# hpc4cmb/flacarray

Hardware: AMD Instinct MI355X
Metric: Msamples/s encode+decode, 4096ch x 1Msamp int32 (higher is better)
Workload: dtype int32

## Files before the change

flacarray_amd/csrc/encode_fused.hpp:

```cpp
#pragma once
#include "encode_kernels.hpp"
#include "quantize_kernels.hpp"

namespace fa {

constexpr int kFSmpWords = 65 * 32;
#ifndef FA_F_SCANW
#define FA_F_SCANW 4
#endif
#ifndef FA_F_RING
#define FA_F_RING 1024
#endif
constexpr int kFRingWords = FA_F_RING;
constexpr int kFRingMask = kFRingWords - 1;
constexpr int kFRingBlocks = kFRingWords / 64;
constexpr int kFRowBlocks = 12;
static_assert(kFRingBlocks - kFRowBlocks - 1 >= 1, "the ring must hold the longest row and a partial block beside what waits to be flushed");
constexpr int kFWaveWords = kFSmpWords + kFRingWords + 4 + 16;
constexpr int kFWaves = 4;
constexpr int kFCrcSlice = 1024;
constexpr int kFCrcXpow = 520;
#ifndef FA_F_SLEEP
#define FA_F_SLEEP 8
#endif
#ifndef FA_F_WBATCH
#define FA_F_WBATCH 4
#endif
#ifndef FA_F_CEIL
#define FA_F_CEIL 1
#endif
#ifndef FA_F_BFLY_N
#define FA_F_BFLY_N 1
#endif
#ifndef FA_F_PARKN
#define FA_F_PARKN 32
#endif
#ifndef FA_F_PARKBLK
#define FA_F_PARKBLK 1
#endif
#ifndef FA_F_PARK
#define FA_F_PARK 1
#endif
#ifndef FA_F_WAVES
#define FA_F_WAVES 3
#endif
constexpr uint32_t kLbSpinLimit = 1u << 22;

struct FusedArgs {
    const int32_t* data;
    const float* f_offsets;
    const float* f_gains;
    int64_t n_stream, stream_size, nframes, total_frames;
    int32_t max_lpc_order, max_porder, precision, pmax_full;
    int32_t tail_bs;
    double escale_full;
    const float* win;
    const uint4* hdr;
    uint8_t* blob;
    int64_t capacity;
    int64_t hb;
    uint32_t* frame_bytes;
    int64_t* frame_abs;
    FrameInfo* info;
    uint32_t* ticket;
    uint32_t* size_pub;
// ... 165 lines not shown
                if ((uint32_t)lane < cnt) {
                    const uint64_t off = prefix + (incl - mine) + (uint64_t)(i / nf + 1u) * (uint64_t)a.hb;
                    __hip_atomic_store(a.off_pub + i, (unsigned long long)off, __ATOMIC_RELAXED, __HIP_MEMORY_SCOPE_AGENT);
#ifdef FA_TIMELINE
                    if (a.info) a.info[i].porder = (int32_t)(uint32_t)__builtin_amdgcn_s_memrealtime();
#endif
                }
                prefix += (uint32_t)__builtin_amdgcn_readlane((int)incl, 63);
                adv += cnt;
            }
            open = open && (cnt == 64u);
        }
        pos += adv;
        if (adv == 0) {
            __builtin_amdgcn_s_sleep(4);
            if (++idle > kLbSpinLimit) {
                if (lane == 0) atomicOr(a.err, 4);
                return;
            }
        } else {
            idle = 0;
        }
    }
    if (lane == 0) *a.total = (int64_t)(prefix + (uint64_t)a.n_stream * (uint64_t)a.hb);
}

#if defined(FA_UNIT_FUSED) || !defined(FA_SPLIT_UNITS)
template <int MLO, bool F32IN = false>
__global__ __launch_bounds__(256) __attribute__((amdgpu_waves_per_eu(MLO > 8 ? 2 : FA_F_WAVES, MLO > 8 ? 2 : FA_F_WAVES))) void encode_fused_kernel(FusedArgs a) {
    static_assert(MLO > 0, "levels 0-2 (fixed predictors, 1152-sample blocks) use the slot path");
    __shared__ __attribute__((aligned(16))) int32_t lds_all[kFWaves * kFWaveWords];
    __shared__ __attribute__((aligned(16))) uint16_t crc_s[kFCrcSlice];
    __shared__ uint32_t ticket_s;

    const int tid = threadIdx.x;
    const int lane = tid & 63;
    const int wave = __builtin_amdgcn_readfirstlane(tid >> 6);
    for (int i = tid; i < kFCrcSlice / 2; i += 256) reinterpret_cast<uint32_t*>(crc_s)[i] = reinterpret_cast<const uint32_t*>(a.crc_tab)[i];
    if (tid == 0) ticket_s = __hip_atomic_fetch_add(a.ticket, 1u, __ATOMIC_RELAXED, __HIP_MEMORY_SCOPE_AGENT);
    __syncthreads();
    const uint32_t ticket = (uint32_t)__builtin_amdgcn_readfirstlane((int)ticket_s);
    if (ticket == 0) {
        if (wave == 0) fused_scanner(a, lane);
        return;
    }
    const int64_t g = (int64_t)(ticket - 1) * kFWaves + wave;
    if (g >= a.total_frames) return;

    int32_t* smp = lds_all + wave * kFWaveWords;
    uint32_t* ring = reinterpret_cast<uint32_t*>(smp + kFSmpWords);
    uint8_t* kpar = reinterpret_cast<uint8_t*>(smp + kFSmpWords + kFRingWords + 4);
    uint32_t* scr = ring;

    const int64_t s = (int64_t)((uint32_t)g / (uint32_t)a.nframes);
    const int64_t f = g - s * a.nframes;
    if (f == a.nframes - 1 && a.tail_bs != kMaxBlock) return;
    constexpr int bs = kMaxBlock;
    const int32_t* src = a.data + (s * a.stream_size + f * (int64_t)bs);
    float q_off = 0.0f, q_gain = 0.0f;
    if constexpr (F32IN) { q_off = a.f_offsets[s]; q_gain = a.f_gains[s]; }
    auto load_row = [&](int j) __attribute__((always_inline)) {
        const int4 v = reinterpret_cast<const int4*>(src)[64 * j + lane];
        if constexpr (F32IN)
            return make_int4(quantise_f32(__int_as_float(v.x), q_off, q_gain), quantise_f32(__int_as_float(v.y), q_off, q_gain),
                             quantise_f32(__int_as_float(v.z), q_off, q_gain), quantise_f32(__int_as_float(v.w), q_off, q_gain));
        else
            return v;
    };
    const float* win = a.win;
    const uint4 fhe = a.hdr[f];
    const uint32_t fh_bits = 32u + ((fhe.w >> 8) & 0xFFu) + ((fhe.w >> 16) & 0xFFu) + (fhe.w >> 24) + 8u;

#define FA_IMAGE_ADDRS                                                                  \
    const int ln_ = lane_id_opaque();                                                   \
    const int K = fsmp_unit(ln_ + 1, 0);                                                \
    const int rowbase = fsmp_unit((ln_ >> 3) + 1, ln_ & 7);                             \
    const int hist7 = fsmp_unit(ln_, 7), hist6 = fsmp_unit(ln_, 6), hist5 = fsmp_unit(ln_, 5); \
    (void)K; (void)rowbase; (void)hist7; (void)hist6; (void)hist5
    constexpr int tailA7 = 32 * 64 + 4 * (7 ^ (64 & 7)), tailA6 = 32 * 64 + 4 * (6 ^ (64 & 7)), tailA5 = 32 * 64 + 4 * (5 ^ (64 & 7));

    FA_STAMP_INIT;
#ifdef FA_TIMELINE
    const uint32_t tl_start_ = (uint32_t)__builtin_amdgcn_s_memrealtime();
#endif
    int4 Bv[8];
    uint32_t orv = 0;
    int mn, mx;
    {
        FA_IMAGE_ADDRS;
        int4 hi[8], lo[8];
// ... 44 lines not shown
        mn >>= wasted;
        mx >>= wasted;
    }
    const bool narrow = (mn >= -(1 << 24)) && (mx < (1 << 24));
    lds_fence();

    FA_STAMP(0);
    const uint64_t verbatim_bits = 8 + (uint64_t)wasted + (uint64_t)bs * (uint64_t)bps;
    int type = 1;
    int order = 0, porder = 0, shift = 0, precision = 0;
    int kbest = 0;
    bool img_is_residual = false;
    bool win_small_l = false, win_small_f = false;
    int fo = -1;
    int32_t qkeep[MLO];
#pragma unroll
    for (int j = 0; j < MLO; ++j) qkeep[j] = 0;
    const int pmax_geo = a.pmax_full;
    auto pmax_for = [&](int pred_order) __attribute__((always_inline)) {
        int pm = pmax_geo;
        while (pm > 0 && (bs >> pm) <= pred_order) pm--;
        return pm;
    };

    auto hist_b = [&](const int4& own, const int4& tail) __attribute__((always_inline)) {
        int4 h;
        h.x = dpp_wave_shr1(tail.x, own.x);
        h.y = dpp_wave_shr1(tail.y, own.y);
        h.z = dpp_wave_shr1(tail.z, own.z);
        h.w = dpp_wave_shr1(tail.w, own.w);
        return h;
    };

    if (__builtin_expect(is_const, 0)) {
        type = 0;
    } else {
        uint64_t best_bits = verbatim_bits;
        double tot0 = 0.0, tot1 = 0.0, tot2 = 0.0, tot3 = 0.0, tot4 = 0.0;
        double mx0 = 0.0, mx1 = 0.0, mx2 = 0.0, mx3 = 0.0, mx4 = 0.0;
        uint64_t hA0 = 0, hA1 = 0, hA2 = 0, hA3 = 0, hA4 = 0;
        double dA0 = 0.0, dA1 = 0.0, dA2 = 0.0, dA3 = 0.0, dA4 = 0.0;
        if (__builtin_expect(narrow, 1)) {
            FA_IMAGE_ADDRS;
            const uint32_t BIAS = 0x80000000u;
            uint32_t s0 = 0, s1 = 0, s2 = 0, s3 = 0, s4 = 0;
            int p1, pe1, pe2, pe3;
            auto seed = [&](const int4& hh) __attribute__((always_inline)) {
                p1 = hh.w;
                pe1 = hh.w - hh.z;
                pe2 = pe1 - (hh.z - hh.y);
                pe3 = pe2 - ((hh.z - hh.y) - (hh.y - hh.x));
            };
            auto group = [&](auto mask_tag, const int4& xv, int gi0) __attribute__((always_inline)) {
                constexpr bool MASK = decltype(mask_tag)::value;
                const int xs[4] = {xv.x, xv.y, xv.z, xv.w};
#pragma unroll
                for (int e = 0; e < 4; ++e) {
                    const int x = xs[e];
                    const int e1 = x - p1, e2 = e1 - pe1, e3 = e2 - pe2;
                    const uint32_t xb = (uint32_t)x ^ BIAS;
                    const uint32_t n0 = sad_u32(xb, BIAS, s0);
                    const uint32_t n1 = sad_u32(xb, (uint32_t)p1 ^ BIAS, s1);
                    const uint32_t n2 = sad_u32((uint32_t)e1 ^ BIAS, (uint32_t)pe1 ^ BIAS, s2);
                    const uint32_t n3 = sad_u32((uint32_t)e2 ^ BIAS, (uint32_t)pe2 ^ BIAS, s3);
                    const uint32_t n4 = sad_u32((uint32_t)e3 ^ BIAS, (uint32_t)pe3 ^ BIAS, s4);
                    if constexpr (MASK) {
                        const int gi = gi0 + e;
                        s0 = n0;
                        s1 = (gi >= 1) ? n1 : s1;
                        s2 = (gi >= 2) ? n2 : s2;
// ... 58 lines not shown
                    mx1 = __builtin_fmax(mx1, a1);
                    mx2 = __builtin_fmax(mx2, a2);
                    mx3 = __builtin_fmax(mx3, a3);
                    mx4 = __builtin_fmax(mx4, a4);
                    p1 = xd; pe1 = e1; pe2 = e2; pe3 = e3;
                }
            };
            seed(*reinterpret_cast<const int4*>(&smp[hist7]));
#pragma unroll 1
            for (int t = 0; t < 8; ++t) group(*reinterpret_cast<const int4*>(&smp[K ^ (4 * t)]), 32 * lane + 4 * t);
            dA0 = tot0; dA1 = tot1; dA2 = tot2; dA3 = tot3; dA4 = tot4;
            seed(hist_b(Bv[7], *reinterpret_cast<const int4*>(&smp[tailA7])));
#pragma unroll
            for (int t = 0; t < 8; ++t) group(Bv[t], 4096);
        }
        FA_STAMP(1);
        {
            double tsum[5] = {tot0, tot1, tot2, tot3, tot4};
            wave_sum_butterfly_n<5>(tsum);
            const double T0 = tsum[0], T1 = tsum[1], T2 = tsum[2], T3 = tsum[3], T4 = tsum[4];
            double M0 = 0.0, M1 = 0.0, M2 = 0.0, M3 = 0.0, M4 = 0.0;
            if (!narrow) {
                M0 = wave_max_f64(mx0); M1 = wave_max_f64(mx1); M2 = wave_max_f64(mx2); M3 = wave_max_f64(mx3);
                M4 = wave_max_f64(mx4);
            }
            const double lim = 2147483647.0;
            double smallest = 1.8446744073709552e19;
            if (M0 <= lim && T0 < smallest) { fo = 0; smallest = T0; }
            if (M1 <= lim && T1 < smallest) { fo = 1; smallest = T1; }
            if (M2 <= lim && T2 < smallest) { fo = 2; smallest = T2; }
            if (M3 <= lim && T3 < smallest) { fo = 3; smallest = T3; }
            if (M4 <= lim && T4 < smallest) { fo = 4; smallest = T4; }
        }
        uint64_t fixA, fixB;
        if (narrow) {
            const uint64_t tA = (fo == 0) ? hA0 : (fo == 1) ? hA1 : (fo == 2) ? hA2 : (fo == 3) ? hA3 : hA4;
            const double tt = (fo == 0) ? tot0 : (fo == 1) ? tot1 : (fo == 2) ? tot2 : (fo == 3) ? tot3 : tot4;
            fixA = tA;
            fixB = (uint64_t)tt - tA;
        } else {
            const double tA = (fo == 0) ? dA0 : (fo == 1) ? dA1 : (fo == 2) ? dA2 : (fo == 3) ? dA3 : dA4;
            const double tt = (fo == 0) ? tot0 : (fo == 1) ? tot1 : (fo == 2) ? tot2 : (fo == 3) ? tot3 : tot4;
            fixA = (uint64_t)tA;
            fixB = (uint64_t)(tt - tA);
        }
        int po_fix = 0, k_fix = 0;
        const int pmax_fix = pmax_for(fo < 0 ? 0 : fo);
        const bool small_fix = __all((fixA < (1u << 24)) && (fixB < (1u << 24)));
        win_small_f = small_fix;
        const bool fuse_search = fo >= 0 && pmax_fix <= 5 && a.max_lpc_order > 0 && small_fix;
        uint64_t est_fix = 0;
        auto apply_fixed = [&]() __attribute__((always_inline)) {
            if (est_fix < best_bits) {
                best_bits = est_fix;
                type = 2;
                order = fo;
                porder = po_fix;
                kbest = k_fix;
            }
        };
        if (__builtin_expect(fo >= 0 && !fuse_search, 0)) {
            uint64_t rb;
            if (pmax_fix <= 5 && small_fix) {
                SplitRiceSearch fs;
                fs.start((uint32_t)fixA, (uint32_t)fixB, fo, pmax_fix, lane);
                fs.gather(); fs.params(); fs.totals();
#pragma unroll
                for (int o = 5; o >= 0; --o) fs.order(o);
                po_fix = fs.bpo; k_fix = fs.kb; rb = fs.best;
            } else {
                rb = split_rice_search_slow(fixA, fixB, fo, pmax_fix, lane, &po_fix, &k_fix);
            }
            est_fix = 8 + (uint64_t)wasted + (uint64_t)fo * (uint64_t)bps + rb;
            apply_fixed();
        }

        FA_STAMP(2);
        int mlo = a.max_lpc_order;
        if (__builtin_expect(mlo > 0, 1)) {
            FA_IMAGE_ADDRS;
            double acc[MLO + 1];
#pragma unroll
            for (int j = 0; j <= MLO; ++j) acc[j] = 0.0;
            SplitRiceSearch fs;
            if (fuse_search) fs.start((uint32_t)fixA, (uint32_t)fixB, fo, pmax_fix, lane);
            double hist[MLO];
            struct WinV { double w[4]; };
            auto load_win = [&](int i0) __attribute__((always_inline)) {
                const float4 f = *reinterpret_cast<const float4*>(win + i0);
                WinV v;
                v.w[0] = (double)f.x; v.w[1] = (double)f.y; v.w[2] = (double)f.z; v.w[3] = (double)f.w;
                return v;
            };
            auto lag_group = [&](const int4& xv, const WinV& wv) __attribute__((always_inline)) {
                const int xs[4] = {xv.x, xv.y, xv.z, xv.w};
#pragma unroll
                for (int e = 0; e < 4; ++e) {
                    const double d = (double)xs[e] * wv.w[e];
                    acc[0] = __builtin_fma(d, d, acc[0]);
#pragma unroll
                    for (int j = 0; j < MLO; ++j) acc[j + 1] = __builtin_fma(d, hist[j], acc[j + 1]);
#pragma unroll
                    for (int j = MLO - 1; j > 0; --j) hist[j] = hist[j - 1];
                    hist[0] = d;
                }
            };
            auto search_stage = [&](int tt) __attribute__((always_inline)) {
                if (!fuse_search) return;
                if (tt == 1) fs.gather();
                if (tt == 3) fs.params();
                if (tt == 5) fs.totals();
                if (tt >= 7 && tt <= 12) fs.order(12 - tt);
// ... 36 lines not shown
#pragma unroll
                for (int t = 0; t < 4; ++t) Bv[4 + t] = pk[64 * t];
            }
#endif
            {
                const int g0 = 2048 + 32 * lane;
                const int4 h7 = hist_b(Bv[7], *reinterpret_cast<const int4*>(&smp[tailA7]));
                const int4 h6 = hist_b(Bv[6], *reinterpret_cast<const int4*>(&smp[tailA6]));
                int4 h5 = make_int4(0, 0, 0, 0);
                if constexpr (MLO > 8) h5 = hist_b(Bv[5], *reinterpret_cast<const int4*>(&smp[tailA5]));
                const int hs[12] = {h7.w, h7.z, h7.y, h7.x, h6.w, h6.z, h6.y, h6.x, h5.w, h5.z, h5.y, h5.x};
#pragma unroll
                for (int j = 0; j < MLO; ++j) hist[j] = (double)hs[j] * (double)win[g0 - 1 - j];
#pragma unroll
                for (int tb = 0; tb < 8; tb += FA_F_WBATCH) {
                    WinV wv[FA_F_WBATCH];
#pragma unroll
                    for (int t = 0; t < FA_F_WBATCH; ++t) wv[t] = load_win(g0 + 4 * (tb + t));
#pragma unroll
                    for (int t = 0; t < FA_F_WBATCH; ++t) {
                        lag_group(Bv[tb + t], wv[t]);
                        search_stage(8 + tb + t);
                    }
                    __builtin_amdgcn_sched_barrier(0);
                }
            }
            FA_STAMP(4);
            if (fuse_search) {
                po_fix = fs.bpo;
                k_fix = fs.kb;
                est_fix = 8 + (uint64_t)wasted + (uint64_t)fo * (uint64_t)bps + (uint64_t)fs.best;
                apply_fixed();
            }
            double autoc[MLO + 1];
#if FA_F_BFLY_N
#pragma unroll
            for (int j = 0; j <= MLO; ++j) autoc[j] = acc[j];
            wave_sum_butterfly_n<MLO + 1>(autoc);
#else
#pragma unroll
            for (int j = 0; j <= MLO; ++j) autoc[j] = wave_sum_butterfly(acc[j]);
#endif

            FA_STAMP(5);
            if (__builtin_expect(autoc[0] != 0.0, 1)) {
                float* coef = reinterpret_cast<float*>(scr);
                double* err = reinterpret_cast<double*>(scr + 160);
                int* meta = reinterpret_cast<int*>(scr + 220);
                if (lane == 0) meta[0] = levinson<MLO>(autoc, mlo, coef, err);
                lds_fence();
                const int usable = meta[0];
                int prec = a.precision;
                int lo;
                {
                    double mybits = 1e300;
                    if (lane < usable) {
                        const double e = err[lane];
                        const double error_scale = a.escale_full;
                        double bpsv;
                        if (e > 0.0) {
                            bpsv = 0.5 * det_log2(error_scale * e);
                            if (!(bpsv >= 0.0)) bpsv = 0.0;
                        } else if (e < 0.0) {
                            bpsv = 1e32;
                        } else {
                            bpsv = 0.0;
                        }
                        mybits = bpsv * (double)(bs - (lane + 1)) + (double)((lane + 1) * (bps + prec));
                    }
                    double bestb = 4294967295.0;
                    int bi = 0;
#pragma unroll
                    for (int o = 0; o < MLO; ++o) {
                        const double b = readlane_f64(mybits, o);
                        if (o < usable && b < bestb) { bestb = b; bi = o; }
                    }
                    lo = bi + 1;
                }
                if (bps <= 17) {
                    const int limp = 32 - bps - ilog2_u64((uint64_t)lo);
                    if (prec > limp) prec = limp;
                }
                int sh = 0;
                int32_t qreg[MLO];
#pragma unroll
                for (int j = 0; j < MLO; ++j) qreg[j] = 0;
                int ok = 0;
                if (prec >= 2) ok = (quantize_coefs_t<MLO>(coef + (lo - 1) * MLO, lo, prec, qreg, &sh) == 0) ? 1 : 0;
                ok = __builtin_amdgcn_readfirstlane(ok);
                sh = __builtin_amdgcn_readfirstlane(sh);
#pragma unroll
                for (int j = 0; j < MLO; ++j) qreg[j] = __builtin_amdgcn_readfirstlane(qreg[j]);
                FA_STAMP(6);
                if (__builtin_expect(ok != 0, 1)) {
                    FA_IMAGE_ADDRS;
                    const double scale = bitsd((uint64_t)(1023 - sh) << 52);
                    double qd[MLO];
#pragma unroll
                    for (int j = 0; j < MLO; ++j) qd[j] = (double)qreg[j] * scale;
                    double tlA = 0.0, tlB = 0.0;
                    double hx[MLO];
                    const int4 a7 = *reinterpret_cast<const int4*>(&smp[hist7]), a6 = *reinterpret_cast<const int4*>(&smp[hist6]);
                    const int4 a5 = *reinterpret_cast<const int4*>(&smp[hist5]);
                    const int4 b7 = hist_b(Bv[7], *reinterpret_cast<const int4*>(&smp[tailA7]));
                    const int4 b6 = hist_b(Bv[6], *reinterpret_cast<const int4*>(&smp[tailA6]));
                    int4 b5 = make_int4(0, 0, 0, 0);
                    if constexpr (MLO > 8) b5 = hist_b(Bv[5], *reinterpret_cast<const int4*>(&smp[tailA5]));
                    lds_fence();
                    auto fold_f64 = [&](double r) __attribute__((always_inline)) {
                        return (int)(uint32_t)__builtin_fabs(__builtin_fma(r, 2.0, 0.5));
                    };
                    auto res_group = [&](auto mask_tag, const int4& xv, int gi0, double& tl) __attribute__((always_inline)) {
                        constexpr bool MASK = decltype(mask_tag)::value;
                        const int xs[4] = {xv.x, xv.y, xv.z, xv.w};
                        int rs[4];
#pragma unroll
                        for (int e = 0; e < 4; ++e) {
                            const double xd = (double)xs[e];
#if FA_F_CEIL
                            double t = xd;
#pragma unroll
                            for (int j = 0; j < MLO; ++j) t = __builtin_fma(-qd[j], hx[j], t);
                            const double r = fa_ceil(t);
#else
                            double sum = 0.0;
#pragma unroll
                            for (int j = 0; j < MLO; ++j) sum = __builtin_fma(qd[j], hx[j], sum);
                            const double pred = fa_floor(sum);
                            const double r = xd - pred;
#endif
                            if constexpr (MASK) {
                                const bool v = (gi0 + e >= lo);
                                tl += v ? fa_fabs(r) : 0.0;
                                rs[e] = v ? fold_f64(r) : xs[e];
                            } else {
                                tl += fa_fabs(r);
                                rs[e] = fold_f64(r);
                            }
#pragma unroll
                            for (int j = MLO - 1; j > 0; --j) hx[j] = hx[j - 1];
                            hx[0] = xd;
                        }
                        return make_int4(rs[0], rs[1], rs[2], rs[3]);
                    };
                    constexpr int kWarmGroups = (MLO + 3) / 4;
                    {
                        const int hs[12] = {a7.w, a7.z, a7.y, a7.x, a6.w, a6.z, a6.y, a6.x, a5.w, a5.z, a5.y, a5.x};
#pragma unroll
                        for (int j = 0; j < MLO; ++j) hx[j] = (double)hs[j];
#pragma unroll
                        for (int t = 0; t < 8; ++t) {
                            int4* px = reinterpret_cast<int4*>(&smp[K ^ (4 * t)]);
                            if (t < kWarmGroups) *px = res_group(std::true_type{}, *px, 32 * lane + 4 * t, tlA);
                            else *px = res_group(std::false_type{}, *px, 0, tlA);
                        }
                    }
                    {
                        const int hs[12] = {b7.w, b7.z, b7.y, b7.x, b6.w, b6.z, b6.y, b6.x, b5.w, b5.z, b5.y, b5.x};
#pragma unroll
                        for (int j = 0; j < MLO; ++j) hx[j] = (double)hs[j];
#pragma unroll
                        for (int t = 0; t < 8; ++t) Bv[t] = res_group(std::false_type{}, Bv[t], 0, tlB);
                    }
                    FA_STAMP(7);
                    img_is_residual = true;
                    const int pmax = pmax_for(lo);
                    int po_l = 0, k_l = 0;
                    uint64_t rbits;
                    const bool small_l = __all((tlA < 16777216.0) && (tlB < 16777216.0));
                    bool lpc_in_range = true;
                    if (__builtin_expect(!small_l, 0)) {
                        bool hit = false;
#pragma unroll 1
                        for (int t = 0; t < 8; ++t) {
                            const int4 ra = *reinterpret_cast<const int4*>(&smp[K ^ (4 * t)]);
                            const int ras[4] = {ra.x, ra.y, ra.z, ra.w};
#pragma unroll
                            for (int e = 0; e < 4; ++e) hit = hit || ((32 * lane + 4 * t + e >= lo) && (uint32_t)ras[e] == 0xffffffffu);
                        }
#pragma unroll
                        for (int t = 0; t < 8; ++t)
                            hit = hit || (uint32_t)Bv[t].x == 0xffffffffu || (uint32_t)Bv[t].y == 0xffffffffu || (uint32_t)Bv[t].z == 0xffffffffu ||
                                  (uint32_t)Bv[t].w == 0xffffffffu;
                        lpc_in_range = !__any(hit);
                    }
                    win_small_l = small_l;
                    if (pmax <= 5 && small_l) {
                        SplitRiceSearch ls;
                        ls.start((uint32_t)tlA, (uint32_t)tlB, lo, pmax, lane);
                        ls.gather(); ls.params(); ls.totals();
#pragma unroll
                        for (int o = 5; o >= 0; --o) ls.order(o);
                        po_l = ls.bpo; k_l = ls.kb; rbits = ls.best;
                    } else {
                        rbits = split_rice_search_slow((uint64_t)tlA, (uint64_t)tlB, lo, pmax, lane, &po_l, &k_l);
                    }
                    if (lpc_in_range) {
                        const uint64_t est = 8 + (uint64_t)wasted + 4 + 5 + (uint64_t)lo * (uint64_t)(prec + bps) + rbits;
                        if (est < best_bits) {
                            best_bits = est;
                            type = 3;
                            order = lo;
                            porder = po_l;
                            kbest = k_l;
                            shift = sh;
                            precision = prec;
#pragma unroll
                            for (int j = 0; j < MLO; ++j) qkeep[j] = qreg[j];
                        }
                    }
                }
                lds_fence();
            }
        }
    }

    FA_STAMP(8);
    const int lane_w = lane_id_opaque();
    auto reload_image = [&]() __attribute__((always_inline)) {
        FA_IMAGE_ADDRS;
#pragma unroll 1
        for (int half = 1; half >= 0; --half) {
#pragma unroll
            for (int j = 0; j < 8; ++j) {
                int4 v = load_row(8 * half + j);
                v.x >>= wasted; v.y >>= wasted; v.z >>= wasted; v.w >>= wasted;
                *reinterpret_cast<int4*>(&smp[rowbase + 256 * j]) = v;
            }
            if (half == 1) {
#pragma unroll
                for (int t = 0; t < 8; ++t) Bv[t] = *reinterpret_cast<const int4*>(&smp[K ^ (4 * t)]);
            }
        }
        lds_fence();
    };
    if (__builtin_expect(type == 2, 0)) {
        if (img_is_residual) {
            reload_image();
            img_is_residual = false;
        }
        {
            FA_IMAGE_ADDRS;
            const int4 ha = *reinterpret_cast<const int4*>(&smp[hist7]);
            const int4 hb2 = hist_b(Bv[7], *reinterpret_cast<const int4*>(&smp[tailA7]));
            lds_fence();
            int64_t x1, x2, x3, x4;
            auto fgroup = [&](const int4& xv, int gi0) __attribute__((always_inline)) {
                const int xs[4] = {xv.x, xv.y, xv.z, xv.w};
                int rs[4];
#pragma unroll
                for (int e = 0; e < 4; ++e) {
                    const int64_t x0 = xs[e];
                    int64_t r;
                    if (order == 0) r = x0;
                    else if (order == 1) r = x0 - x1;
                    else if (order == 2) r = x0 - 2 * x1 + x2;
                    else if (order == 3) r = x0 - 3 * x1 + 3 * x2 - x3;
                    else r = x0 - 4 * x1 + 6 * x2 - 4 * x3 + x4;
                    rs[e] = (gi0 + e >= order) ? rice_fold((int)r) : xs[e];
                    x4 = x3; x3 = x2; x2 = x1; x1 = x0;
                }
                return make_int4(rs[0], rs[1], rs[2], rs[3]);
            };
            x1 = ha.w; x2 = ha.z; x3 = ha.y; x4 = ha.x;
#pragma unroll 1
            for (int t = 0; t < 8; ++t) {
                int4* px = reinterpret_cast<int4*>(&smp[K ^ (4 * t)]);
                *px = fgroup(*px, 32 * lane_w + 4 * t);
            }
            x1 = hb2.w; x2 = hb2.z; x3 = hb2.y; x4 = hb2.x;
#pragma unroll
// ... 40 lines not shown
        };
        if (__builtin_expect((type == 3) ? win_small_l : win_small_f, 1)) size_lane(std::false_type{});
        else size_lane(std::true_type{});
        bitsA += (8 - kWarmGroupsS) * 4 * (kA + 1u);
        bitsB += 32u * (kB + 1u);
        if (((uint32_t)lane_w & (cpp - 1u)) == 0u || cpp > 64u) {
            if (cpp <= 64u) { bitsA += (uint32_t)plen; bitsB += (uint32_t)plen; }
            else if (lane_w == 0) bitsA += (uint32_t)plen;
        }
        uint32_t rA = bitsA, rB = bitsB;
        rA += (uint32_t)xchg_i32<0>((int)rA); rB += (uint32_t)xchg_i32<0>((int)rB);
        rA += (uint32_t)xchg_i32<1>((int)rA); rB += (uint32_t)xchg_i32<1>((int)rB);
        rA += (uint32_t)xchg_i32<2>((int)rA); rB += (uint32_t)xchg_i32<2>((int)rB);
        const bool row_over = __any((rA > (uint32_t)kRowCapBits) || (rB > (uint32_t)kRowCapBits));
        const uint64_t exact = 6 + wave_sum_u64((uint64_t)bitsA + bitsB) + 8 + (uint64_t)wasted + (uint64_t)order * (uint64_t)bps +
                               ((type == 3) ? (4 + 5 + (uint64_t)order * (uint64_t)precision) : 0);
        if (row_over || exact > verbatim_bits) {
            type = 1;
            order = 0;
            porder = 0;
        }
        sub_bits = (uint32_t)exact;
    }
    if (type == 0) sub_bits = 8u + (uint32_t)wasted + (uint32_t)bps;
    if (type == 1) sub_bits = (uint32_t)verbatim_bits;
    const uint32_t total_bytes = ((fh_bits + sub_bits + 7u) >> 3) + 2u;
    const uint32_t L = total_bytes - 2u;

    FA_STAMP(9);
    const uint32_t F = (uint32_t)a.total_frames;
    const uint32_t gu = (uint32_t)g;
#ifdef FA_TIMELINE
    if (lane_w == 0 && a.info) {
        a.info[g].wasted = (int32_t)tl_start_;
        a.info[g].shift = (int32_t)(uint32_t)__builtin_amdgcn_s_memrealtime();
        __builtin_amdgcn_s_waitcnt(0);
    }
#endif
    if (lane_w == 0) {
        __hip_atomic_store(a.size_pub + gu, 0x80000000u | total_bytes, __ATOMIC_RELAXED, __HIP_MEMORY_SCOPE_AGENT);
        a.frame_bytes[g] = total_bytes;
    }
    (void)F;
#ifndef FA_TIMELINE
    if (lane_w == 0 && a.info) {
        FrameInfo fi;
        fi.type = type;
        fi.order = (type >= 2) ? order : 0;
        fi.porder = (type >= 2) ? porder : 0;
        fi.wasted = wasted;
        fi.shift = (type == 3) ? shift : 0;
        fi.precision = (type == 3) ? precision : 0;
        fi.nbytes = (int32_t)total_bytes;
        fi.blocksize = bs;
        a.info[g] = fi;
    }
#endif

#ifdef FA_F_ANALYSIS_ONLY
    if (lane_w == 0) a.frame_abs[g] = g * (int64_t)kSlotBytes + (s + 1) * a.hb;
    return;
#endif
    kpar[lane_w] = (uint8_t)kbest;
    for (int i = lane_w; i < kFRingWords; i += 64) ring[i] = 0;
    if (lane_w == 0) ring[kFRingWords] = 0;
    lds_fence();
// ... 487 lines not shown
```

Before: 203,000.

## Batch Levinson solves of all block waves onto the last-arriving wave

Each wave publishes its autocorrelation to shared memory, and the last wave to arrive solves the Levinson recursion and coefficient quantisation for all four frames in parallel, 16 lanes per frame. Meanwhile the other waves run the fixed-predictor analysis, then poll with a bounded sleep for the result, falling back to a local solve if it never arrives. This aims to hide the serial single-lane Levinson latency behind the fixed analysis, at the cost of intra-block coupling, polling overhead and extra LDS. It also adds an order-0 fixed path that folds residuals in place instead of recomputing them.

Result: faster. 208,300 (median of 6 runs) (+2.6%).

```diff
diff --git a/flacarray_amd/csrc/encode_fused.hpp b/flacarray_amd/csrc/encode_fused.hpp
--- a/flacarray_amd/csrc/encode_fused.hpp
+++ b/flacarray_amd/csrc/encode_fused.hpp
@@ -31,6 +31,18 @@
 #endif
 #ifndef FA_F_BFLY_N
 #define FA_F_BFLY_N 1
+#endif
+#ifndef FA_F_SHLEV
+#define FA_F_SHLEV 1
+#endif
+#ifndef FA_F_SHLEV_MAXMLO
+#define FA_F_SHLEV_MAXMLO 12
+#endif
+#ifndef FA_F_SHPOLL
+#define FA_F_SHPOLL 256
+#endif
+#ifndef FA_F_SHSLEEP
+#define FA_F_SHSLEEP 4
 #endif
 #ifndef FA_F_PARKN
 #define FA_F_PARKN 32
@@ -262,12 +274,23 @@
     __shared__ __attribute__((aligned(16))) int32_t lds_all[kFWaves * kFWaveWords];
     __shared__ __attribute__((aligned(16))) uint16_t crc_s[kFCrcSlice];
     __shared__ uint32_t ticket_s;
+    constexpr bool SHLEV = (FA_F_SHLEV != 0) && (MLO <= FA_F_SHLEV_MAXMLO);
+    static_assert(!SHLEV || kFRingWords >= 256 * kFWaves, "the solving wave works in its idle bit ring: 256 words per problem");
+    __shared__ double lev_in[SHLEV ? kFWaves : 1][MLO + 1];
+    __shared__ int lev_bps[SHLEV ? kFWaves : 1];
+    __shared__ int lev_out[SHLEV ? kFWaves : 1][MLO + 4];
+    __shared__ uint32_t lev_rdy[SHLEV ? kFWaves : 1];
+    __shared__ uint32_t lev_cnt;
 
     const int tid = threadIdx.x;
     const int lane = tid & 63;
     const int wave = __builtin_amdgcn_readfirstlane(tid >> 6);
     for (int i = tid; i < kFCrcSlice / 2; i += 256) reinterpret_cast<uint32_t*>(crc_s)[i] = reinterpret_cast<const uint32_t*>(a.crc_tab)[i];
     if (tid == 0) ticket_s = __hip_atomic_fetch_add(a.ticket, 1u, __ATOMIC_RELAXED, __HIP_MEMORY_SCOPE_AGENT);
+    if constexpr (SHLEV) {
+        if (tid == 0) lev_cnt = 0;
+        if (tid < kFWaves) lev_rdy[tid] = 0;
+    }
     __syncthreads();
     const uint32_t ticket = (uint32_t)__builtin_amdgcn_readfirstlane((int)ticket_s);
     if (ticket == 0) {
@@ -275,17 +298,118 @@
         return;
     }
     const int64_t g = (int64_t)(ticket - 1) * kFWaves + wave;
-    if (g >= a.total_frames) return;
 
     int32_t* smp = lds_all + wave * kFWaveWords;
     uint32_t* ring = reinterpret_cast<uint32_t*>(smp + kFSmpWords);
     uint8_t* kpar = reinterpret_cast<uint8_t*>(smp + kFSmpWords + kFRingWords + 4);
     uint32_t* scr = ring;
+    constexpr int bs = kMaxBlock;
+
+    auto lpc_solve = [&](auto grp_tag, const double (&ac)[MLO + 1], int fbps, uint32_t* wscr, int sub, int& wok, int& wlo, int& wprec,
+                         int& wsh, int32_t (&wq)[MLO]) __attribute__((always_inline)) {
+        constexpr int GRP = decltype(grp_tag)::value;
+        float* coef = reinterpret_cast<float*>(wscr);
+        double* err = reinterpret_cast<double*>(wscr + 160);
+        int* meta = reinterpret_cast<int*>(wscr + 220);
+        if (sub == 0) meta[0] = levinson<MLO>(ac, a.max_lpc_order, coef, err);
+        lds_fence();
+        const int usable = meta[0];
+        wprec = a.precision;
+        {
+            double mybits = 1e300;
+            if (sub < usable) {
+                const double e = err[sub];
+                const double error_scale = a.escale_full;
+                double bpsv;
+                if (e > 0.0) {
+                    bpsv = 0.5 * det_log2(error_scale * e);
+                    if (!(bpsv >= 0.0)) bpsv = 0.0;
+                } else if (e < 0.0) {
+                    bpsv = 1e32;
+                } else {
+                    bpsv = 0.0;
+                }
+                mybits = bpsv * (double)(bs - (sub + 1)) + (double)((sub + 1) * (fbps + wprec));
+            }
+            double bestb = 4294967295.0;
+            int bi = 0;
+            if constexpr (GRP == 64) {
+#pragma unroll
+                for (int o = 0; o < MLO; ++o) {
+                    const double b = readlane_f64(mybits, o);
+                    if (o < usable && b < bestb) { bestb = b; bi = o; }
+                }
+            } else {
+                double* mbv = reinterpret_cast<double*>(wscr + 224);
+                if (sub < MLO) mbv[sub] = mybits;
+                lds_fence();
+#pragma unroll
+                for (int o = 0; o < MLO; ++o) {
+                    const double b = mbv[o];
+                    if (o < usable && b < bestb) { bestb = b; bi = o; }
+                }
+            }
+            wlo = bi + 1;
+        }
+        if (fbps <= 17) {
+            const int limp = 32 - fbps - ilog2_u64((uint64_t)wlo);
+            if (wprec > limp) wprec = limp;
+        }
+        wsh = 0;
+#pragma unroll
+        for (int j = 0; j < MLO; ++j) wq[j] = 0;
+        wok = 0;
+        if (wprec >= 2) wok = (quantize_coefs_t<MLO>(coef + (wlo - 1) * MLO, wlo, wprec, wq, &wsh) == 0) ? 1 : 0;
+    };
+    auto shlev_announce = [&](bool cand, int fbps, const double* ac) __attribute__((always_inline)) {
+        const int ln = lane_id_opaque();
+        if (ln == 0) {
+            if (cand) {
+#pragma unroll
+                for (int j = 0; j <= MLO; ++j) lev_in[wave][j] = ac[j];
+            }
+            lev_bps[wave] = cand ? fbps : -1;
+        }
+        lds_fence();
+        uint32_t before = 0;
+        if (ln == 0) before = __hip_atomic_fetch_add(&lev_cnt, 1u, __ATOMIC_RELAXED, __HIP_MEMORY_SCOPE_WORKGROUP);
+        lds_fence();
+        if ((uint32_t)__builtin_amdgcn_readfirstlane((int)before) != (uint32_t)(kFWaves - 1)) return;
+        const int fr = ln >> 4, sub = ln & 15;
+        const int fbps_w = lev_bps[fr];
+        double acw[MLO + 1];
+#pragma unroll
+        for (int j = 0; j <= MLO; ++j) acw[j] = lev_in[fr][j];
+        if (fbps_w < 0) {
+            acw[0] = 1.0;
+#pragma unroll
+            for (int j = 1; j <= MLO; ++j) acw[j] = 0.0;
+        }
+        int wok, wlo, wprec, wsh;
+        int32_t wq[MLO];
+        lpc_solve(std::integral_constant<int, 16>{}, acw, fbps_w, scr + 256 * fr, sub, wok, wlo, wprec, wsh, wq);
+        if (sub == 0) {
+            lev_out[fr][0] = wok; lev_out[fr][1] = wlo; lev_out[fr][2] = wprec; lev_out[fr][3] = wsh;
+#pragma unroll
+            for (int j = 0; j < MLO; ++j) lev_out[fr][4 + j] = wq[j];
+        }
+        lds_fence();
+        if (sub == 0) __hip_atomic_store(&lev_rdy[fr], 1u, __ATOMIC_RELAXED, __HIP_MEMORY_SCOPE_WORKGROUP);
+        lds_fence();
+    };
+    if constexpr (SHLEV) {
+        bool mine = g < a.total_frames;
+        if (mine && a.tail_bs != kMaxBlock) mine = ((uint32_t)g % (uint32_t)a.nframes) != (uint32_t)(a.nframes - 1);
+        if (__builtin_expect(!mine, 0)) {
+            shlev_announce(false, 0, nullptr);
+            return;
+        }
+    }
+    if (g >= a.total_frames) return;
 
     const int64_t s = (int64_t)((uint32_t)g / (uint32_t)a.nframes);
     const int64_t f = g - s * a.nframes;
     if (f == a.nframes - 1 && a.tail_bs != kMaxBlock) return;
-    constexpr int bs = kMaxBlock;
     const int32_t* src = a.data + (s * a.stream_size + f * (int64_t)bs);
     float q_off = 0.0f, q_gain = 0.0f;
     if constexpr (F32IN) { q_off = a.f_offsets[s]; q_gain = a.f_gains[s]; }
@@ -396,10 +520,22 @@
         return h;
     };
 
-    if (__builtin_expect(is_const, 0)) {
-        type = 0;
-    } else {
-        uint64_t best_bits = verbatim_bits;
+    uint64_t best_bits = verbatim_bits;
+    bool lpc_cand = false;
+    double autoc[MLO + 1];
+    uint64_t fixA = 0, fixB = 0, est_fix = 0;
+    int po_fix = 0, k_fix = 0, pmax_fix = 0;
+    bool fuse_search = false;
+    auto apply_fixed = [&]() __attribute__((always_inline)) {
+        if (est_fix < best_bits) {
+            best_bits = est_fix;
+            type = 2;
+            order = fo;
+            porder = po_fix;
+            kbest = k_fix;
+        }
+    };
+    auto fixed_analysis = [&]() __attribute__((always_inline)) {
         double tot0 = 0.0, tot1 = 0.0, tot2 = 0.0, tot3 = 0.0, tot4 = 0.0;
         double mx0 = 0.0, mx1 = 0.0, mx2 = 0.0, mx3 = 0.0, mx4 = 0.0;
         uint64_t hA0 = 0, hA1 = 0, hA2 = 0, hA3 = 0, hA4 = 0;
@@ -524,7 +660,6 @@
             if (M3 <= lim && T3 < smallest) { fo = 3; smallest = T3; }
             if (M4 <= lim && T4 < smallest) { fo = 4; smallest = T4; }
         }
-        uint64_t fixA, fixB;
         if (narrow) {
             const uint64_t tA = (fo == 0) ? hA0 : (fo == 1) ? hA1 : (fo == 2) ? hA2 : (fo == 3) ? hA3 : hA4;
             const double tt = (fo == 0) ? tot0 : (fo == 1) ? tot1 : (fo == 2) ? tot2 : (fo == 3) ? tot3 : tot4;
@@ -536,22 +671,11 @@
             fixA = (uint64_t)tA;
             fixB = (uint64_t)(tt - tA);
         }
-        int po_fix = 0, k_fix = 0;
-        const int pmax_fix = pmax_for(fo < 0 ? 0 : fo);
+        pmax_fix = pmax_for(fo < 0 ? 0 : fo);
         const bool small_fix = __all((fixA < (1u << 24)) && (fixB < (1u << 24)));
         win_small_f = small_fix;
-        const bool fuse_search = fo >= 0 && pmax_fix <= 5 && a.max_lpc_order > 0 && small_fix;
-        uint64_t est_fix = 0;
-        auto apply_fixed = [&]() __attribute__((always_inline)) {
-            if (est_fix < best_bits) {
-                best_bits = est_fix;
-                type = 2;
-                order = fo;
-                porder = po_fix;
-                kbest = k_fix;
-            }
-        };
-        if (__builtin_expect(fo >= 0 && !fuse_search, 0)) {
+        fuse_search = !SHLEV && fo >= 0 && pmax_fix <= 5 && a.max_lpc_order > 0 && small_fix;
+        if (__builtin_expect(fo >= 0 && !fuse_search, SHLEV ? 1 : 0)) {
             uint64_t rb;
             if (pmax_fix <= 5 && small_fix) {
                 SplitRiceSearch fs;
@@ -566,10 +690,14 @@
             est_fix = 8 + (uint64_t)wasted + (uint64_t)fo * (uint64_t)bps + rb;
             apply_fixed();
         }
-
         FA_STAMP(2);
-        int mlo = a.max_lpc_order;
-        if (__builtin_expect(mlo > 0, 1)) {
+    };
+
+    if (__builtin_expect(is_const, 0)) {
+        type = 0;
+    } else {
+        if constexpr (!SHLEV) fixed_analysis();
+        if (__builtin_expect(a.max_lpc_order > 0, 1)) {
             FA_IMAGE_ADDRS;
             double acc[MLO + 1];
 #pragma unroll
@@ -672,7 +800,6 @@
                 est_fix = 8 + (uint64_t)wasted + (uint64_t)fo * (uint64_t)bps + (uint64_t)fs.best;
                 apply_fixed();
             }
-            double autoc[MLO + 1];
 #if FA_F_BFLY_N
 #pragma unroll
             for (int j = 0; j <= MLO; ++j) autoc[j] = acc[j];
@@ -681,183 +808,180 @@
 #pragma unroll
             for (int j = 0; j <= MLO; ++j) autoc[j] = wave_sum_butterfly(acc[j]);
 #endif
-
-            FA_STAMP(5);
-            if (__builtin_expect(autoc[0] != 0.0, 1)) {
-                float* coef = reinterpret_cast<float*>(scr);
-                double* err = reinterpret_cast<double*>(scr + 160);
-                int* meta = reinterpret_cast<int*>(scr + 220);
-                if (lane == 0) meta[0] = levinson<MLO>(autoc, mlo, coef, err);
-                lds_fence();
-                const int usable = meta[0];
-                int prec = a.precision;
-                int lo;
-                {
-                    double mybits = 1e300;
-                    if (lane < usable) {
-                        const double e = err[lane];
-                        const double error_scale = a.escale_full;
-                        double bpsv;
-                        if (e > 0.0) {
-                            bpsv = 0.5 * det_log2(error_scale * e);
-                            if (!(bpsv >= 0.0)) bpsv = 0.0;
-                        } else if (e < 0.0) {
-                            bpsv = 1e32;
-                        } else {
-                            bpsv = 0.0;
-                        }
-                        mybits = bpsv * (double)(bs - (lane + 1)) + (double)((lane + 1) * (bps + prec));
-                    }
-                    double bestb = 4294967295.0;
-                    int bi = 0;
-#pragma unroll
-                    for (int o = 0; o < MLO; ++o) {
-                        const double b = readlane_f64(mybits, o);
-                        if (o < usable && b < bestb) { bestb = b; bi = o; }
-                    }
-                    lo = bi + 1;
-                }
-                if (bps <= 17) {
-                    const int limp = 32 - bps - ilog2_u64((uint64_t)lo);
-                    if (prec > limp) prec = limp;
-                }
-                int sh = 0;
-                int32_t qreg[MLO];
-#pragma unroll
-                for (int j = 0; j < MLO; ++j) qreg[j] = 0;
-                int ok = 0;
-                if (prec >= 2) ok = (quantize_coefs_t<MLO>(coef + (lo - 1) * MLO, lo, prec, qreg, &sh) == 0) ? 1 : 0;
-                ok = __builtin_amdgcn_readfirstlane(ok);
-                sh = __builtin_amdgcn_readfirstlane(sh);
-#pragma unroll
-                for (int j = 0; j < MLO; ++j) qreg[j] = __builtin_amdgcn_readfirstlane(qreg[j]);
-                FA_STAMP(6);
-                if (__builtin_expect(ok != 0, 1)) {
-                    FA_IMAGE_ADDRS;
-                    const double scale = bitsd((uint64_t)(1023 - sh) << 52);
-                    double qd[MLO];
-#pragma unroll
-                    for (int j = 0; j < MLO; ++j) qd[j] = (double)qreg[j] * scale;
-                    double tlA = 0.0, tlB = 0.0;
-                    double hx[MLO];
-                    const int4 a7 = *reinterpret_cast<const int4*>(&smp[hist7]), a6 = *reinterpret_cast<const int4*>(&smp[hist6]);
-                    const int4 a5 = *reinterpret_cast<const int4*>(&smp[hist5]);
-                    const int4 b7 = hist_b(Bv[7], *reinterpret_cast<const int4*>(&smp[tailA7]));
-                    const int4 b6 = hist_b(Bv[6], *reinterpret_cast<const int4*>(&smp[tailA6]));
-                    int4 b5 = make_int4(0, 0, 0, 0);
-                    if constexpr (MLO > 8) b5 = hist_b(Bv[5], *reinterpret_cast<const int4*>(&smp[tailA5]));
-                    lds_fence();
-                    auto fold_f64 = [&](double r) __attribute__((always_inline)) {
-                        return (int)(uint32_t)__builtin_fabs(__builtin_fma(r, 2.0, 0.5));
-                    };
-                    auto res_group = [&](auto mask_tag, const int4& xv, int gi0, double& tl) __attribute__((always_inline)) {
-                        constexpr bool MASK = decltype(mask_tag)::value;
-                        const int xs[4] = {xv.x, xv.y, xv.z, xv.w};
-                        int rs[4];
-#pragma unroll
-                        for (int e = 0; e < 4; ++e) {
-                            const double xd = (double)xs[e];
+            lpc_cand = (autoc[0] != 0.0);
+        }
+    }
+
+    FA_STAMP(5);
+    int ok = 0, lo = 0, prec = a.precision, sh = 0;
+    int32_t qreg[MLO];
+#pragma unroll
+    for (int j = 0; j < MLO; ++j) qreg[j] = 0;
+    if constexpr (SHLEV) {
+        shlev_announce(lpc_cand, bps, autoc);
+        FA_STAMP(6);
+        if (!is_const) fixed_analysis();
+        if (lpc_cand) {
+#ifdef FA_STAMPS
+            const unsigned long long tw0_ = fa_memtime();
+#endif
+            uint32_t up = 0, polls = 0;
+            for (;;) {
+                up = (uint32_t)__builtin_amdgcn_readfirstlane((int)__hip_atomic_load(&lev_rdy[wave], __ATOMIC_RELAXED, __HIP_MEMORY_SCOPE_WORKGROUP));
+                if (up != 0 || ++polls > (uint32_t)FA_F_SHPOLL) break;
+                __builtin_amdgcn_s_sleep(FA_F_SHSLEEP);
+            }
+            lds_fence();
+#ifdef FA_STAMPS
+            if (lane_id_opaque() == 0 && a.stamps && (blockIdx.x & 63) == 0) {
+                atomicAdd(&a.stamps[17], fa_memtime() - tw0_);
+                atomicAdd(&a.stamps[18], (unsigned long long)polls);
+                atomicAdd(&a.stamps[19], up != 0 ? 0ULL : 1ULL);
+                atomicAdd(&a.stamps[20], 1ULL);
+            }
+#endif
+            if (__builtin_expect(up != 0, 1)) {
+                ok = lev_out[wave][0]; lo = lev_out[wave][1]; prec = lev_out[wave][2]; sh = lev_out[wave][3];
+#pragma unroll
+                for (int j = 0; j < MLO; ++j) qreg[j] = lev_out[wave][4 + j];
+            } else {
+                lpc_solve(std::integral_constant<int, 64>{}, autoc, bps, scr, lane_id_opaque(), ok, lo, prec, sh, qreg);
+            }
+        }
+    } else {
+        if (lpc_cand) lpc_solve(std::integral_constant<int, 64>{}, autoc, bps, scr, lane, ok, lo, prec, sh, qreg);
+        FA_STAMP(6);
+    }
+    ok = __builtin_amdgcn_readfirstlane(ok);
+    lo = __builtin_amdgcn_readfirstlane(lo);
+    prec = __builtin_amdgcn_readfirstlane(prec);
+    sh = __builtin_amdgcn_readfirstlane(sh);
+#pragma unroll
+    for (int j = 0; j < MLO; ++j) qreg[j] = __builtin_amdgcn_readfirstlane(qreg[j]);
+    if (__builtin_expect(lpc_cand && ok != 0, 1)) {
+        FA_IMAGE_ADDRS;
+        const double scale = bitsd((uint64_t)(1023 - sh) << 52);
+        double qd[MLO];
+#pragma unroll
+        for (int j = 0; j < MLO; ++j) qd[j] = (double)qreg[j] * scale;
+        double tlA = 0.0, tlB = 0.0;
+        double hx[MLO];
+        const int4 a7 = *reinterpret_cast<const int4*>(&smp[hist7]), a6 = *reinterpret_cast<const int4*>(&smp[hist6]);
+        const int4 a5 = *reinterpret_cast<const int4*>(&smp[hist5]);
+        const int4 b7 = hist_b(Bv[7], *reinterpret_cast<const int4*>(&smp[tailA7]));
+        const int4 b6 = hist_b(Bv[6], *reinterpret_cast<const int4*>(&smp[tailA6]));
+        int4 b5 = make_int4(0, 0, 0, 0);
+        if constexpr (MLO > 8) b5 = hist_b(Bv[5], *reinterpret_cast<const int4*>(&smp[tailA5]));
+        lds_fence();
+        auto fold_f64 = [&](double r) __attribute__((always_inline)) {
+            return (int)(uint32_t)__builtin_fabs(__builtin_fma(r, 2.0, 0.5));
+        };
+        auto res_group = [&](auto mask_tag, const int4& xv, int gi0, double& tl) __attribute__((always_inline)) {
+            constexpr bool MASK = decltype(mask_tag)::value;
+            const int xs[4] = {xv.x, xv.y, xv.z, xv.w};
+            int rs[4];
+#pragma unroll
+            for (int e = 0; e < 4; ++e) {
+                const double xd = (double)xs[e];
 #if FA_F_CEIL
-                            double t = xd;
-#pragma unroll
-                            for (int j = 0; j < MLO; ++j) t = __builtin_fma(-qd[j], hx[j], t);
-                            const double r = fa_ceil(t);
+                double t = xd;
+#pragma unroll
+                for (int j = 0; j < MLO; ++j) t = __builtin_fma(-qd[j], hx[j], t);
+                const double r = fa_ceil(t);
 #else
-                            double sum = 0.0;
-#pragma unroll
-                            for (int j = 0; j < MLO; ++j) sum = __builtin_fma(qd[j], hx[j], sum);
-                            const double pred = fa_floor(sum);
-                            const double r = xd - pred;
-#endif
-                            if constexpr (MASK) {
-                                const bool v = (gi0 + e >= lo);
-                                tl += v ? fa_fabs(r) : 0.0;
-                                rs[e] = v ? fold_f64(r) : xs[e];
-                            } else {
-                                tl += fa_fabs(r);
-                                rs[e] = fold_f64(r);
-                            }
-#pragma unroll
-                            for (int j = MLO - 1; j > 0; --j) hx[j] = hx[j - 1];
-                            hx[0] = xd;
-                        }
-                        return make_int4(rs[0], rs[1], rs[2], rs[3]);
-                    };
-                    constexpr int kWarmGroups = (MLO + 3) / 4;
-                    {
-                        const int hs[12] = {a7.w, a7.z, a7.y, a7.x, a6.w, a6.z, a6.y, a6.x, a5.w, a5.z, a5.y, a5.x};
-#pragma unroll
-                        for (int j = 0; j < MLO; ++j) hx[j] = (double)hs[j];
-#pragma unroll
-                        for (int t = 0; t < 8; ++t) {
-                            int4* px = reinterpret_cast<int4*>(&smp[K ^ (4 * t)]);
-                            if (t < kWarmGroups) *px = res_group(std::true_type{}, *px, 32 * lane + 4 * t, tlA);
-                            else *px = res_group(std::false_type{}, *px, 0, tlA);
-                        }
-                    }
-                    {
-                        const int hs[12] = {b7.w, b7.z, b7.y, b7.x, b6.w, b6.z, b6.y, b6.x, b5.w, b5.z, b5.y, b5.x};
-#pragma unroll
-                        for (int j = 0; j < MLO; ++j) hx[j] = (double)hs[j];
-#pragma unroll
-                        for (int t = 0; t < 8; ++t) Bv[t] = res_group(std::false_type{}, Bv[t], 0, tlB);
-                    }
-                    FA_STAMP(7);
-                    img_is_residual = true;
-                    const int pmax = pmax_for(lo);
-                    int po_l = 0, k_l = 0;
-                    uint64_t rbits;
-                    const bool small_l = __all((tlA < 16777216.0) && (tlB < 16777216.0));
-                    bool lpc_in_range = true;
-                    if (__builtin_expect(!small_l, 0)) {
-                        bool hit = false;
+                double sum = 0.0;
+#pragma unroll
+                for (int j = 0; j < MLO; ++j) sum = __builtin_fma(qd[j], hx[j], sum);
+                const double pred = fa_floor(sum);
+                const double r = xd - pred;
+#endif
+                if constexpr (MASK) {
+                    const bool v = (gi0 + e >= lo);
+                    tl += v ? fa_fabs(r) : 0.0;
+                    rs[e] = v ? fold_f64(r) : xs[e];
+                } else {
+                    tl += fa_fabs(r);
+                    rs[e] = fold_f64(r);
+                }
+#pragma unroll
+                for (int j = MLO - 1; j > 0; --j) hx[j] = hx[j - 1];
+                hx[0] = xd;
+            }
+            return make_int4(rs[0], rs[1], rs[2], rs[3]);
+        };
+        constexpr int kWarmGroups = (MLO + 3) / 4;
+        {
+            const int hs[12] = {a7.w, a7.z, a7.y, a7.x, a6.w, a6.z, a6.y, a6.x, a5.w, a5.z, a5.y, a5.x};
+#pragma unroll
+            for (int j = 0; j < MLO; ++j) hx[j] = (double)hs[j];
+#pragma unroll
+            for (int t = 0; t < 8; ++t) {
+                int4* px = reinterpret_cast<int4*>(&smp[K ^ (4 * t)]);
+                if (t < kWarmGroups) *px = res_group(std::true_type{}, *px, 32 * lane + 4 * t, tlA);
+                else *px = res_group(std::false_type{}, *px, 0, tlA);
+            }
+        }
+        {
+            const int hs[12] = {b7.w, b7.z, b7.y, b7.x, b6.w, b6.z, b6.y, b6.x, b5.w, b5.z, b5.y, b5.x};
+#pragma unroll
+            for (int j = 0; j < MLO; ++j) hx[j] = (double)hs[j];
+#pragma unroll
+            for (int t = 0; t < 8; ++t) Bv[t] = res_group(std::false_type{}, Bv[t], 0, tlB);
+        }
+        FA_STAMP(7);
+        img_is_residual = true;
+        const int pmax = pmax_for(lo);
+        int po_l = 0, k_l = 0;
+        uint64_t rbits;
+        const bool small_l = __all((tlA < 16777216.0) && (tlB < 16777216.0));
+        bool lpc_in_range = true;
+        if (__builtin_expect(!small_l, 0)) {
+            bool hit = false;
 #pragma unroll 1
-                        for (int t = 0; t < 8; ++t) {
-                            const int4 ra = *reinterpret_cast<const int4*>(&smp[K ^ (4 * t)]);
-                            const int ras[4] = {ra.x, ra.y, ra.z, ra.w};
-#pragma unroll
-                            for (int e = 0; e < 4; ++e) hit = hit || ((32 * lane + 4 * t + e >= lo) && (uint32_t)ras[e] == 0xffffffffu);
-                        }
-#pragma unroll
-                        for (int t = 0; t < 8; ++t)
-                            hit = hit || (uint32_t)Bv[t].x == 0xffffffffu || (uint32_t)Bv[t].y == 0xffffffffu || (uint32_t)Bv[t].z == 0xffffffffu ||
-                                  (uint32_t)Bv[t].w == 0xffffffffu;
-                        lpc_in_range = !__any(hit);
-                    }
-                    win_small_l = small_l;
-                    if (pmax <= 5 && small_l) {
-                        SplitRiceSearch ls;
-                        ls.start((uint32_t)tlA, (uint32_t)tlB, lo, pmax, lane);
-                        ls.gather(); ls.params(); ls.totals();
-#pragma unroll
-                        for (int o = 5; o >= 0; --o) ls.order(o);
-                        po_l = ls.bpo; k_l = ls.kb; rbits = ls.best;
-                    } else {
-                        rbits = split_rice_search_slow((uint64_t)tlA, (uint64_t)tlB, lo, pmax, lane, &po_l, &k_l);
-                    }
-                    if (lpc_in_range) {
-                        const uint64_t est = 8 + (uint64_t)wasted + 4 + 5 + (uint64_t)lo * (uint64_t)(prec + bps) + rbits;
-                        if (est < best_bits) {
-                            best_bits = est;
-                            type = 3;
-                            order = lo;
-                            porder = po_l;
-                            kbest = k_l;
-                            shift = sh;
-                            precision = prec;
-#pragma unroll
-                            for (int j = 0; j < MLO; ++j) qkeep[j] = qreg[j];
-                        }
-                    }
-                }
-                lds_fence();
-            }
-        }
-    }
+            for (int t = 0; t < 8; ++t) {
+                const int4 ra = *reinterpret_cast<const int4*>(&smp[K ^ (4 * t)]);
+                const int ras[4] = {ra.x, ra.y, ra.z, ra.w};
+#pragma unroll
+                for (int e = 0; e < 4; ++e) hit = hit || ((32 * lane + 4 * t + e >= lo) && (uint32_t)ras[e] == 0xffffffffu);
+            }
+#pragma unroll
+            for (int t = 0; t < 8; ++t)
+                hit = hit || (uint32_t)Bv[t].x == 0xffffffffu || (uint32_t)Bv[t].y == 0xffffffffu || (uint32_t)Bv[t].z == 0xffffffffu ||
+                      (uint32_t)Bv[t].w == 0xffffffffu;
+            lpc_in_range = !__any(hit);
+        }
+        win_small_l = small_l;
+        if (pmax <= 5 && small_l) {
+            SplitRiceSearch ls;
+            ls.start((uint32_t)tlA, (uint32_t)tlB, lo, pmax, lane);
+            ls.gather(); ls.params(); ls.totals();
+#pragma unroll
+            for (int o = 5; o >= 0; --o) ls.order(o);
+            po_l = ls.bpo; k_l = ls.kb; rbits = ls.best;
+        } else {
+            rbits = split_rice_search_slow((uint64_t)tlA, (uint64_t)tlB, lo, pmax, lane, &po_l, &k_l);
+        }
+        if (lpc_in_range) {
+            const uint64_t est = 8 + (uint64_t)wasted + 4 + 5 + (uint64_t)lo * (uint64_t)(prec + bps) + rbits;
+            if (est < best_bits) {
+                best_bits = est;
+                type = 3;
+                order = lo;
+                porder = po_l;
+                kbest = k_l;
+                shift = sh;
+                precision = prec;
+#pragma unroll
+                for (int j = 0; j < MLO; ++j) qkeep[j] = qreg[j];
+            }
+        }
+    }
+    lds_fence();
 
     FA_STAMP(8);
     const int lane_w = lane_id_opaque();
-    auto reload_image = [&]() __attribute__((always_inline)) {
+    auto reload_image = [&](auto fold_tag) __attribute__((always_inline)) {
+        constexpr bool FOLD = decltype(fold_tag)::value;
         FA_IMAGE_ADDRS;
 #pragma unroll 1
         for (int half = 1; half >= 0; --half) {
@@ -865,6 +989,7 @@
             for (int j = 0; j < 8; ++j) {
                 int4 v = load_row(8 * half + j);
                 v.x >>= wasted; v.y >>= wasted; v.z >>= wasted; v.w >>= wasted;
+                if constexpr (FOLD) { v.x = rice_fold(v.x); v.y = rice_fold(v.y); v.z = rice_fold(v.z); v.w = rice_fold(v.w); }
                 *reinterpret_cast<int4*>(&smp[rowbase + 256 * j]) = v;
             }
             if (half == 1) {
@@ -874,9 +999,25 @@
         }
         lds_fence();
     };
-    if (__builtin_expect(type == 2, 0)) {
+    if (__builtin_expect(type == 2 && order == 0, 0)) {
         if (img_is_residual) {
-            reload_image();
+            reload_image(std::true_type{});
+        } else {
+            FA_IMAGE_ADDRS;
+#pragma unroll
+            for (int t = 0; t < 8; ++t) {
+                int4* px = reinterpret_cast<int4*>(&smp[K ^ (4 * t)]);
+                int4 v = *px;
+                v.x = rice_fold(v.x); v.y = rice_fold(v.y); v.z = rice_fold(v.z); v.w = rice_fold(v.w);
+                *px = v;
+                Bv[t].x = rice_fold(Bv[t].x); Bv[t].y = rice_fold(Bv[t].y); Bv[t].z = rice_fold(Bv[t].z); Bv[t].w = rice_fold(Bv[t].w);
+            }
+            lds_fence();
+        }
+        img_is_residual = true;
+    } else if (__builtin_expect(type == 2, 0)) {
+        if (img_is_residual) {
+            reload_image(std::false_type{});
             img_is_residual = false;
         }
         {
@@ -983,6 +1124,8 @@
     const uint32_t gu = (uint32_t)g;
 #ifdef FA_TIMELINE
     if (lane_w == 0 && a.info) {
+        a.info[g].type = type;
+        a.info[g].order = (type >= 2) ? order : 0;
         a.info[g].wasted = (int32_t)tl_start_;
         a.info[g].shift = (int32_t)(uint32_t)__builtin_amdgcn_s_memrealtime();
         __builtin_amdgcn_s_waitcnt(0);
```
